# yondonfu/ai-rtc-agent

Measured on NVIDIA H100. Metric: frames/sec at 512x512 SD-Turbo img2img (1-step, stream-batch 1), higher is better.
Workload: dtype f16

## Files before the change

### ai-rtc-agent_b200/csrc/ptx.cuh

```cuda
#pragma once
#include <cuda.h>
#include <cuda_fp16.h>
#include <cuda_runtime.h>
#include <stdint.h>
#include <stdio.h>

namespace b2 {

__device__ __forceinline__ uint32_t smem_u32(const void* p) {
    return static_cast<uint32_t>(__cvta_generic_to_shared(p));
}

__device__ __forceinline__ uint64_t globaltimer_ns() {
    uint64_t t;
    asm volatile("mov.u64 %0, %%globaltimer;" : "=l"(t));
    return t;
}

__device__ __forceinline__ void mbar_init(uint64_t* bar, uint32_t count) {
    asm volatile("mbarrier.init.shared::cta.b64 [%0], %1;" ::"r"(smem_u32(bar)), "r"(count));
}
__device__ __forceinline__ void fence_mbar_init() {
    asm volatile("fence.mbarrier_init.release.cluster;" ::: "memory");
}
__device__ __forceinline__ void mbar_expect_tx(uint64_t* bar, uint32_t bytes) {
    asm volatile("mbarrier.arrive.expect_tx.shared::cta.b64 _, [%0], %1;" ::"r"(smem_u32(bar)),
                 "r"(bytes)
                 : "memory");
}
__device__ __forceinline__ void mbar_arrive(uint64_t* bar) {
    asm volatile("mbarrier.arrive.shared::cta.b64 _, [%0];" ::"r"(smem_u32(bar)) : "memory");
}
__device__ __forceinline__ bool mbar_try_wait(uint64_t* bar, uint32_t parity) {
    uint32_t ok;
    asm volatile(
        "{\n\t"
        ".reg .pred P;\n\t"
        "mbarrier.try_wait.parity.shared::cta.b64 P, [%1], %2;\n\t"
        "selp.u32 %0, 1, 0, P;\n\t"
        "}\n"
        : "=r"(ok)
        : "r"(smem_u32(bar)), "r"(parity)
        : "memory");
    return ok != 0;
}
#ifndef B2_WAIT_TIMEOUT_NS
#define B2_WAIT_TIMEOUT_NS 4000000000ull
#endif
__device__ __forceinline__ void mbar_wait(uint64_t* bar, uint32_t parity) {
    if (mbar_try_wait(bar, parity)) return;
    uint64_t t0 = 0;
    uint32_t spins = 0;
    while (!mbar_try_wait(bar, parity)) {
        if ((++spins & 0x3ff) == 0) {
            const uint64_t now = globaltimer_ns();
            if (t0 == 0) t0 = now;
            else if (now - t0 > B2_WAIT_TIMEOUT_NS) __trap();
        }
    }
}

__device__ __forceinline__ void mbar_arrive_remote(uint32_t cluster_addr) {
    asm volatile("mbarrier.arrive.shared::cluster.b64 _, [%0];" ::"r"(cluster_addr) : "memory");
}

__device__ __forceinline__ void fence_proxy_async_smem() {
    asm volatile("fence.proxy.async.shared::cta;" ::: "memory");
}

__device__ __forceinline__ void cluster_sync_all() {
    asm volatile("barrier.cluster.arrive.release.aligned;" ::: "memory");
    asm volatile("barrier.cluster.wait.acquire.aligned;" ::: "memory");
}
__device__ __forceinline__ void cluster_arrive_relaxed() { asm volatile("barrier.cluster.arrive.relaxed.aligned;" ::: "memory"); }
__device__ __forceinline__ void cluster_wait() { asm volatile("barrier.cluster.wait.aligned;" ::: "memory"); }
__device__ __forceinline__ uint32_t cluster_ctarank() {
    uint32_t r;
    asm volatile("mov.u32 %0, %%cluster_ctarank;" : "=r"(r));
    return r;
}
__device__ __forceinline__ uint32_t dsmem_map(uint32_t local_smem_addr, uint32_t rank) {
    uint32_t r;
    asm volatile("mapa.shared::cluster.u32 %0, %1, %2;" : "=r"(r) : "r"(local_smem_addr), "r"(rank));
    return r;
}
__device__ __forceinline__ void dsmem_st_f2(uint32_t cluster_addr, float x, float y) {
    asm volatile("st.shared::cluster.v2.f32 [%0], {%1, %2};" ::"r"(cluster_addr), "f"(x), "f"(y) : "memory");
}
__device__ __forceinline__ float4 dsmem_ld_f4(uint32_t cluster_addr) {
    float4 v;
    asm volatile("ld.shared::cluster.v4.f32 {%0, %1, %2, %3}, [%4];"
                 : "=f"(v.x), "=f"(v.y), "=f"(v.z), "=f"(v.w)
                 : "r"(cluster_addr)
                 : "memory");
    return v;
}

__device__ __forceinline__ void tma_prefetch_desc(const CUtensorMap* m) {
    asm volatile("prefetch.tensormap [%0];" ::"l"(reinterpret_cast<uint64_t>(m)) : "memory");
}
__device__ __forceinline__ void tma_load_2d(void* smem_dst, const CUtensorMap* m, uint64_t* bar,
                                            int c0, int c1) {
    asm volatile(
        "cp.async.bulk.tensor.2d.shared::cluster.global.mbarrier::complete_tx::bytes [%0], [%1, {%3, "
        "%4}], [%2];" ::"r"(smem_u32(smem_dst)),
        "l"(reinterpret_cast<uint64_t>(m)), "r"(smem_u32(bar)), "r"(c0), "r"(c1)
        : "memory");
}
__device__ __forceinline__ void tma_load_4d(void* smem_dst, const CUtensorMap* m, uint64_t* bar,
                                            int c0, int c1, int c2, int c3) {
    asm volatile(
        "cp.async.bulk.tensor.4d.shared::cluster.global.mbarrier::complete_tx::bytes [%0], [%1, {%3, "
        "%4, %5, %6}], [%2];" ::"r"(smem_u32(smem_dst)),
        "l"(reinterpret_cast<uint64_t>(m)), "r"(smem_u32(bar)), "r"(c0), "r"(c1), "r"(c2), "r"(c3)
        : "memory");
}

__device__ __forceinline__ void tma_load_2d_mc(void* smem_dst, const CUtensorMap* m, uint64_t* bar, int c0, int c1, uint16_t cta_mask) {
    asm volatile(
        "cp.async.bulk.tensor.2d.shared::cluster.global.mbarrier::complete_tx::bytes.multicast::cluster [%0], [%1, {%3, %4}], [%2], "
        "%5;" ::"r"(smem_u32(smem_dst)),
        "l"(reinterpret_cast<uint64_t>(m)), "r"(smem_u32(bar)), "r"(c0), "r"(c1), "h"(cta_mask)
        : "memory");
}

__device__ __forceinline__ void wgmma_fence() { asm volatile("wgmma.fence.sync.aligned;" ::: "memory"); }
__device__ __forceinline__ void wgmma_commit() { asm volatile("wgmma.commit_group.sync.aligned;" ::: "memory"); }
template <int N>
__device__ __forceinline__ void wgmma_wait() { asm volatile("wgmma.wait_group.sync.aligned %0;" ::"n"(N) : "memory"); }
template <int N>
__device__ __forceinline__ void wgmma_fence_regs(float (&d)[N]) {
#pragma unroll
    for (int i = 0; i < N; ++i) asm volatile("" : "+f"(d[i])::"memory");
}

__device__ __forceinline__ uint64_t make_kmajor_sw128_desc(uint32_t smem_addr, uint32_t sbo = 1024) {
    uint64_t d = 0;
    d |= (uint64_t)((smem_addr & 0x3ffff) >> 4);
    d |= (uint64_t)1 << 16;
    d |= (uint64_t)(sbo >> 4) << 32;
    d |= (uint64_t)1 << 62;
    return d;
}

}
```

### ai-rtc-agent_b200/csrc/tconv.cu

```cuda
#include "tconv.cuh"

#include <cudaTypedefs.h>
#include <stdlib.h>

#include "epilogue.cuh"
#include "launch.cuh"
#include "ptx.cuh"

namespace b2 {

constexpr uint32_t TC_WTILE = TC_C * TC_C * 2;
constexpr uint32_t TC_HALO_BYTES = (TC_TW + 2) * (TC_TH + 2) * TC_C * 2;

__global__ void __launch_bounds__(TC_THREADS, 1) tconv_kernel(const __grid_constant__ TconvParams p) {
    extern __shared__ uint8_t smem_raw[];
    uint8_t* smem = reinterpret_cast<uint8_t*>((reinterpret_cast<uintptr_t>(smem_raw) + 1023) & ~static_cast<uintptr_t>(1023));
    const int warp = threadIdx.x >> 5;
    const int lane = threadIdx.x & 31;
    uint8_t* sW = smem;
    uint8_t* sA = smem + 9 * TC_WTILE;
    uint64_t* w_full = reinterpret_cast<uint64_t*>(sA + (size_t)p.nbuf * p.abuf_bytes);
    uint64_t* a_full = w_full + 1;
    uint64_t* a_empty = a_full + TC_MAX_ABUF;

    if (threadIdx.x == TC_CONS) {
        tma_prefetch_desc(&p.tmA);
        tma_prefetch_desc(&p.tmB);
        mbar_init(w_full, 1);
        for (int s = 0; s < p.nbuf; ++s) {
            mbar_init(&a_full[s], 1);
            mbar_init(&a_empty[s], 4);
        }
        fence_mbar_init();
    }
    __syncthreads();
    if (threadIdx.x == TC_CONS) {
        mbar_expect_tx(w_full, 9 * TC_WTILE);
        for (int tap = 0; tap < 9; ++tap) tma_load_2d(sW + tap * TC_WTILE, &p.tmB, w_full, tap * TC_C, 0);
    }
    pdl_launch_dependents();
    pdl_wait();

    const int tiles_per_img = p.tiles_w * p.tiles_h;
    if (warp == TC_CONS / 32) {
        if (lane == 0) {
            int slot = 0;
            uint32_t phase = 0;
            for (int mt = blockIdx.x; mt < p.num_tiles; mt += gridDim.x) {
                const int tiw = mt % p.tiles_w, tih = (mt / p.tiles_w) % p.tiles_h, n0 = mt / tiles_per_img;
                mbar_wait(&a_empty[slot], phase ^ 1);
                mbar_expect_tx(&a_full[slot], TC_HALO_BYTES);
                tma_load_4d(sA + (size_t)slot * p.abuf_bytes, &p.tmA, &a_full[slot], 0, tiw * TC_TW - 1, tih * TC_TH - 1, n0);
                if (++slot == p.nbuf) {
                    slot = 0;
                    phase ^= 1;
                }
            }
        }
    } else {
        const int wg = warp >> 2;
        const uint32_t sa_base = smem_u32(sA);
        const uint64_t db0 = make_kmajor_sw128_desc(smem_u32(sW));
        constexpr int pitch = TC_TW + 2;
        const int rq = (warp & 3) * 16 + (lane >> 2);
        const IgEpilogue& e = p.epi;
        mbar_wait(w_full, 0);
        for (int it = wg, mt = blockIdx.x + wg * gridDim.x; mt < p.num_tiles; it += 2, mt += 2 * gridDim.x) {
            const int slot = it % p.nbuf;
            mbar_wait(&a_full[slot], (uint32_t)(it / p.nbuf) & 1u);
            float acc[2][TC_C / 2];
#pragma unroll
            for (int m = 0; m < 2; ++m)
#pragma unroll
                for (int i = 0; i < TC_C / 2; ++i) acc[m][i] = 0.f;
            wgmma_fence_regs(acc[0]);
            wgmma_fence_regs(acc[1]);
            wgmma_fence();
            const uint32_t a0 = sa_base + (uint32_t)slot * p.abuf_bytes;
#pragma unroll
            for (int tap = 0; tap < 9; ++tap) {
                const uint64_t db = db0 + (uint64_t)(tap * (TC_WTILE >> 4));
#pragma unroll
                for (int m = 0; m < 2; ++m) {
                    const uint32_t sa = a0 + (uint32_t)((8 * m + tap / 3) * pitch + tap % 3) * 128u;
                    const uint64_t da = make_kmajor_sw128_desc(sa, pitch * 128);
#pragma unroll
                    for (int k = 0; k < 4; ++k) Wgmma<TC_C>::ss(acc[m], da + 2 * k, db + 2 * k, 1u);
                }
            }
            wgmma_commit();
            wgmma_wait<0>();
            wgmma_fence_regs(acc[0]);
            wgmma_fence_regs(acc[1]);
            if (lane == 0) mbar_arrive(&a_empty[slot]);
            const int tiw = mt % p.tiles_w, tih = (mt / p.tiles_w) % p.tiles_h, n0 = mt / tiles_per_img;
#pragma unroll
            for (int m = 0; m < 2; ++m) {
                EpiRow rw[2];
#pragma unroll
                for (int h = 0; h < 2; ++h) {
                    const int r = 64 * m + rq + 8 * h;
                    const int hh = tih * TC_TH + (r >> 3), ww = tiw * TC_TW + (r & 7);
                    rw[h].ok = (hh < p.Ho) && (ww < p.Wo);
                    rw[h].orow = ((long)n0 * p.Ho + hh) * p.Wo + ww;
                    rw[h].b = n0;
                    rw[h].mu = 0.f;
                    rw[h].rstd = 1.f;
                }
                epi_frag<TC_C>(e, acc[m], rw, 0, false, lane);
            }
        }
    }
}

bool tconv_eligible(const IgemmDesc& d) {
    const IgEpilogue& e = d.epi;
    return d.nseg == 1 && d.ntap[0] == 9 && d.stride <= 1 && !d.swap && d.src[0].C == TC_C && e.n_valid == TC_C &&
           d.w_rows >= TC_C && d.w_ld == 9 * TC_C && d.src[0].H == d.Ho && d.src[0].W == d.Wo && d.src[0].N == d.Nb &&
           !(e.flags & (IG_GEGLU | IG_SPLITK | IG_SILU)) && (e.ldc & 7) == 0 && (!e.res || (e.ldr & 7) == 0) && (e.colbias_bstride & 3) == 0 &&
           (d.src[0].ld & 7) == 0 && !(reinterpret_cast<uintptr_t>(d.src[0].ptr) & 15) && !(reinterpret_cast<uintptr_t>(d.w) & 15) &&
           !(reinterpret_cast<uintptr_t>(e.out) & 15) && !(reinterpret_cast<uintptr_t>(e.res) & 15) &&
           !(reinterpret_cast<uintptr_t>(e.colbias) & 15);
}

int igemm_encode_act_map(CUtensorMap* m, const ActView& a, int box_c, int box_w, int box_h, int box_n, int estride);
int igemm_encode_w_map(CUtensorMap* m, const __half* w, int rows, int ld, int box_rows);

int tconv_plan(const IgemmDesc& d, TconvPlan* plan) {
    *plan = TconvPlan{};
    if (!tconv_eligible(d)) {
        b2_set_error("tconv: needs a stride-1 3x3 convolution with 64 input and 64 output channels and a vectorisable epilogue");
        return -1;
    }
    TconvParams& p = plan->p;
    p.tiles_w = (d.Wo + TC_TW - 1) / TC_TW;
    p.tiles_h = (d.Ho + TC_TH - 1) / TC_TH;
    p.num_tiles = p.tiles_w * p.tiles_h * d.Nb;
    p.Wo = d.Wo; p.Ho = d.Ho; p.Nb = d.Nb;
    static const char* nb_env = getenv("B2_TCONV_NBUF");
    p.nbuf = nb_env ? atoi(nb_env) : 4;
    if (p.nbuf < 2) p.nbuf = 2;
    if (p.nbuf > TC_MAX_ABUF) p.nbuf = TC_MAX_ABUF;
    p.nbuf &= ~1;
    p.abuf_bytes = (TC_HALO_BYTES + 1023u) & ~1023u;
    p.epi = d.epi;
    if (igemm_encode_act_map(&p.tmA, d.src[0], TC_C, TC_TW + 2, TC_TH + 2, 1, 1)) return -1;
    if (igemm_encode_w_map(&p.tmB, d.w, d.w_rows, d.w_ld, TC_C)) return -1;
    const int sms = b2_device_sms();
    plan->grid = dim3(p.num_tiles < sms ? p.num_tiles : sms, 1, 1);
    plan->smem = 9 * (size_t)TC_WTILE + (size_t)p.nbuf * p.abuf_bytes + 1024  + 512 ;
    plan->rows_total = (long)d.Nb * d.Ho * d.Wo;
    return 0;
}

int tconv_init() {
    static bool done = false;
    if (!done) {
        cudaError_t e = cudaFuncSetAttribute(tconv_kernel, cudaFuncAttributeMaxDynamicSharedMemorySize, 227 * 1024);
        if (e != cudaSuccess) {
            b2_set_error("cudaFuncSetAttribute(tconv): %s", cudaGetErrorString(e));
            return -1;
        }
        done = true;
    }
    return 0;
}

int tconv_launch(const TconvPlan& plan, cudaStream_t stream) {
    if (tconv_init()) return -1;
    cudaError_t e = launch_k(tconv_kernel, plan.grid, dim3(TC_THREADS), plan.smem, stream, 1, plan.p);
    if (e != cudaSuccess) {
        b2_set_error("tconv launch: %s", cudaGetErrorString(e));
        return -1;
    }
    return 0;
}

}
```

### ai-rtc-agent_b200/csrc/tconv.cuh

```cuda
#pragma once
#include "igemm.cuh"

namespace b2 {

constexpr int TC_CONS = 256;
constexpr int TC_THREADS = TC_CONS + 32;
constexpr int TC_TW = 8, TC_TH = 16;
constexpr int TC_C = 64;
constexpr int TC_MAX_ABUF = 6;

struct TconvParams {
    CUtensorMap tmA;
    CUtensorMap tmB;
    int tiles_w, tiles_h, num_tiles;
    int Wo, Ho, Nb;
    int nbuf;
    uint32_t abuf_bytes;
    IgEpilogue epi;
};

struct TconvPlan {
    TconvParams p;
    dim3 grid;
    size_t smem;
    long rows_total;
};

bool tconv_eligible(const IgemmDesc& d);
int tconv_plan(const IgemmDesc& d, TconvPlan* plan);
int tconv_launch(const TconvPlan& plan, cudaStream_t stream);
int tconv_init();

}
```

Measured before the change: 173.0.

## Stage tconv epilogue through swizzled smem and write via TMA stores with residual TMA loads

Replaces the per-thread global epilogue of the 64-channel 3x3 conv kernel with a staged epilogue: fragments are written into swizzled shared memory, the residual tile is fetched by TMA into the same staging buffer, and output is written back with 4D TMA bulk stores. The wgmma loop is reordered so each half-tile commits separately, letting the first half's epilogue overlap the second half's MMAs. It also narrows eligibility (no per-batch bias, colsum, rowstat or second output) and caps A buffers at 4 to fit the staging space. This targets uncoalesced global stores and residual loads, at the cost of extra shared memory, named barriers and fewer A pipeline stages.

```diff
diff --git a/ai-rtc-agent_b200/csrc/ptx.cuh b/ai-rtc-agent_b200/csrc/ptx.cuh
--- a/ai-rtc-agent_b200/csrc/ptx.cuh
+++ b/ai-rtc-agent_b200/csrc/ptx.cuh
@@ -116,6 +116,21 @@
         : "memory");
 }
 
+__device__ __forceinline__ void tma_store_4d(const CUtensorMap* m, const void* smem_src, int c0, int c1, int c2, int c3) {
+    asm volatile("cp.async.bulk.tensor.4d.global.shared::cta.bulk_group [%0, {%2, %3, %4, %5}], [%1];" ::"l"(reinterpret_cast<uint64_t>(m)),
+                 "r"(smem_u32(smem_src)), "r"(c0), "r"(c1), "r"(c2), "r"(c3)
+                 : "memory");
+}
+__device__ __forceinline__ void bulk_commit_group() { asm volatile("cp.async.bulk.commit_group;" ::: "memory"); }
+template <int N>
+__device__ __forceinline__ void bulk_wait_group_read() { asm volatile("cp.async.bulk.wait_group.read %0;" ::"n"(N) : "memory"); }
+template <int N>
+__device__ __forceinline__ void bulk_wait_group() { asm volatile("cp.async.bulk.wait_group %0;" ::"n"(N) : "memory"); }
+
+__device__ __forceinline__ void named_bar_sync(int id, int count) {
+    asm volatile("bar.sync %0, %1;" ::"r"(id), "r"(count) : "memory");
+}
+
 __device__ __forceinline__ void tma_load_2d_mc(void* smem_dst, const CUtensorMap* m, uint64_t* bar, int c0, int c1, uint16_t cta_mask) {
     asm volatile(
         "cp.async.bulk.tensor.2d.shared::cluster.global.mbarrier::complete_tx::bytes.multicast::cluster [%0], [%1, {%3, %4}], [%2], "
diff --git a/ai-rtc-agent_b200/csrc/tconv.cu b/ai-rtc-agent_b200/csrc/tconv.cu
--- a/ai-rtc-agent_b200/csrc/tconv.cu
+++ b/ai-rtc-agent_b200/csrc/tconv.cu
@@ -3,34 +3,42 @@
 #include <cudaTypedefs.h>
 #include <stdlib.h>
 
-#include "epilogue.cuh"
 #include "launch.cuh"
 #include "ptx.cuh"
+#include "wgmma.cuh"
 
 namespace b2 {
 
 constexpr uint32_t TC_WTILE = TC_C * TC_C * 2;
 constexpr uint32_t TC_HALO_BYTES = (TC_TW + 2) * (TC_TH + 2) * TC_C * 2;
+constexpr uint32_t TC_SLAB_BYTES = 64 * TC_C * 2;
+constexpr uint32_t TC_STG_BYTES = 2 * TC_SLAB_BYTES;
 
 __global__ void __launch_bounds__(TC_THREADS, 1) tconv_kernel(const __grid_constant__ TconvParams p) {
     extern __shared__ uint8_t smem_raw[];
-    uint8_t* smem = reinterpret_cast<uint8_t*>((reinterpret_cast<uintptr_t>(smem_raw) + 1023) & ~static_cast<uintptr_t>(1023));
+    uint8_t* smem = smem_raw + ((1024u - (smem_u32(smem_raw) & 1023u)) & 1023u);
     const int warp = threadIdx.x >> 5;
     const int lane = threadIdx.x & 31;
     uint8_t* sW = smem;
     uint8_t* sA = smem + 9 * TC_WTILE;
-    uint64_t* w_full = reinterpret_cast<uint64_t*>(sA + (size_t)p.nbuf * p.abuf_bytes);
+    uint8_t* sS = sA + (size_t)p.nbuf * p.abuf_bytes;
+    uint64_t* w_full = reinterpret_cast<uint64_t*>(sS + 2 * TC_STG_BYTES);
     uint64_t* a_full = w_full + 1;
     uint64_t* a_empty = a_full + TC_MAX_ABUF;
+    uint64_t* r_full = a_empty + TC_MAX_ABUF;
 
     if (threadIdx.x == TC_CONS) {
         tma_prefetch_desc(&p.tmA);
         tma_prefetch_desc(&p.tmB);
+        tma_prefetch_desc(&p.tmO);
+        if (p.epi.res) tma_prefetch_desc(&p.tmR);
         mbar_init(w_full, 1);
         for (int s = 0; s < p.nbuf; ++s) {
             mbar_init(&a_full[s], 1);
             mbar_init(&a_empty[s], 4);
         }
+        mbar_init(&r_full[0], 1);
+        mbar_init(&r_full[1], 1);
         fence_mbar_init();
     }
     __syncthreads();
@@ -59,13 +67,25 @@
         }
     } else {
         const int wg = warp >> 2;
+        const bool leader = (threadIdx.x & 127) == 0;
         const uint32_t sa_base = smem_u32(sA);
         const uint64_t db0 = make_kmajor_sw128_desc(smem_u32(sW));
         constexpr int pitch = TC_TW + 2;
         const int rq = (warp & 3) * 16 + (lane >> 2);
         const IgEpilogue& e = p.epi;
+        const bool has_bias = e.colbias != nullptr, has_res = e.res != nullptr, relu = (e.flags & IG_RELU) != 0;
+        float bias[TC_C / 4];
+#pragma unroll
+        for (int j = 0; j < TC_C / 8; ++j) {
+            const float2 b = has_bias ? *reinterpret_cast<const float2*>(e.colbias + 8 * j + 2 * (lane & 3)) : make_float2(0.f, 0.f);
+            bias[2 * j] = b.x;
+            bias[2 * j + 1] = b.y;
+        }
+        uint8_t* stg = sS + wg * TC_STG_BYTES;
+        uint8_t* stg_t = stg + rq * 128 + 4 * (lane & 3);
         mbar_wait(w_full, 0);
         for (int it = wg, mt = blockIdx.x + wg * gridDim.x; mt < p.num_tiles; it += 2, mt += 2 * gridDim.x) {
+            const int tiw = mt % p.tiles_w, tih = (mt / p.tiles_w) % p.tiles_h, n0 = mt / tiles_per_img;
             const int slot = it % p.nbuf;
             mbar_wait(&a_full[slot], (uint32_t)(it / p.nbuf) & 1u);
             float acc[2][TC_C / 2];
@@ -78,38 +98,72 @@
             wgmma_fence();
             const uint32_t a0 = sa_base + (uint32_t)slot * p.abuf_bytes;
 #pragma unroll
-            for (int tap = 0; tap < 9; ++tap) {
-                const uint64_t db = db0 + (uint64_t)(tap * (TC_WTILE >> 4));
-#pragma unroll
-                for (int m = 0; m < 2; ++m) {
+            for (int m = 0; m < 2; ++m) {
+#pragma unroll
+                for (int tap = 0; tap < 9; ++tap) {
+                    const uint64_t db = db0 + (uint64_t)(tap * (TC_WTILE >> 4));
                     const uint32_t sa = a0 + (uint32_t)((8 * m + tap / 3) * pitch + tap % 3) * 128u;
                     const uint64_t da = make_kmajor_sw128_desc(sa, pitch * 128);
 #pragma unroll
                     for (int k = 0; k < 4; ++k) Wgmma<TC_C>::ss(acc[m], da + 2 * k, db + 2 * k, 1u);
                 }
-            }
-            wgmma_commit();
-            wgmma_wait<0>();
-            wgmma_fence_regs(acc[0]);
-            wgmma_fence_regs(acc[1]);
-            if (lane == 0) mbar_arrive(&a_empty[slot]);
-            const int tiw = mt % p.tiles_w, tih = (mt / p.tiles_w) % p.tiles_h, n0 = mt / tiles_per_img;
+                wgmma_commit();
+            }
+            if (leader) {
+                bulk_wait_group_read<0>();
+                if (has_res) {
+                    mbar_expect_tx(&r_full[wg], TC_STG_BYTES);
+                    tma_load_4d(stg, &p.tmR, &r_full[wg], 0, tiw * TC_TW, tih * TC_TH, n0);
+                } else {
+                    mbar_arrive(&r_full[wg]);
+                }
+            }
 #pragma unroll
             for (int m = 0; m < 2; ++m) {
-                EpiRow rw[2];
-#pragma unroll
-                for (int h = 0; h < 2; ++h) {
-                    const int r = 64 * m + rq + 8 * h;
-                    const int hh = tih * TC_TH + (r >> 3), ww = tiw * TC_TW + (r & 7);
-                    rw[h].ok = (hh < p.Ho) && (ww < p.Wo);
-                    rw[h].orow = ((long)n0 * p.Ho + hh) * p.Wo + ww;
-                    rw[h].b = n0;
-                    rw[h].mu = 0.f;
-                    rw[h].rstd = 1.f;
-                }
-                epi_frag<TC_C>(e, acc[m], rw, 0, false, lane);
-            }
-        }
+                if (m == 0) {
+                    wgmma_wait<1>();
+                    wgmma_fence_regs(acc[0]);
+                    mbar_wait(&r_full[wg], (uint32_t)(it >> 1) & 1u);
+                } else {
+                    wgmma_wait<0>();
+                    wgmma_fence_regs(acc[1]);
+                    if (lane == 0) mbar_arrive(&a_empty[slot]);
+                }
+#pragma unroll
+                for (int j = 0; j < TC_C / 8; ++j) {
+#pragma unroll
+                    for (int h = 0; h < 2; ++h) {
+                        __half2* sp = reinterpret_cast<__half2*>(stg_t + (64 * m + 8 * h) * 128 + ((j ^ (lane >> 2)) << 4));
+                        float x0 = acc[m][4 * j + 2 * h], x1 = acc[m][4 * j + 2 * h + 1];
+                        if (has_bias) {
+                            x0 += bias[2 * j];
+                            x1 += bias[2 * j + 1];
+                        }
+                        if (e.acc_scale != 1.0f) {
+                            x0 *= e.acc_scale;
+                            x1 *= e.acc_scale;
+                        }
+                        if (has_res) {
+                            const float2 f = __half22float2(*sp);
+                            x0 = fmaf(e.res_scale, f.x, x0);
+                            x1 = fmaf(e.res_scale, f.y, x1);
+                        }
+                        if (relu) {
+                            x0 = fmaxf(x0, 0.f);
+                            x1 = fmaxf(x1, 0.f);
+                        }
+                        *sp = __floats2half2_rn(x0, x1);
+                    }
+                }
+                fence_proxy_async_smem();
+                named_bar_sync(1 + wg, 128);
+                if (leader) {
+                    tma_store_4d(&p.tmO, stg + m * TC_SLAB_BYTES, 0, tiw * TC_TW, tih * TC_TH + 8 * m, n0);
+                    bulk_commit_group();
+                }
+            }
+        }
+        if (leader) bulk_wait_group<0>();
     }
 }
 
@@ -117,7 +171,8 @@
     const IgEpilogue& e = d.epi;
     return d.nseg == 1 && d.ntap[0] == 9 && d.stride <= 1 && !d.swap && d.src[0].C == TC_C && e.n_valid == TC_C &&
            d.w_rows >= TC_C && d.w_ld == 9 * TC_C && d.src[0].H == d.Ho && d.src[0].W == d.Wo && d.src[0].N == d.Nb &&
-           !(e.flags & (IG_GEGLU | IG_SPLITK | IG_SILU)) && (e.ldc & 7) == 0 && (!e.res || (e.ldr & 7) == 0) && (e.colbias_bstride & 3) == 0 &&
+           !(e.flags & (IG_GEGLU | IG_SPLITK | IG_SILU)) && !e.colsum && !e.rowstat_out && !e.out2 && (e.ldc & 7) == 0 &&
+           (!e.res || (e.ldr & 7) == 0) && e.colbias_bstride == 0 &&
            (d.src[0].ld & 7) == 0 && !(reinterpret_cast<uintptr_t>(d.src[0].ptr) & 15) && !(reinterpret_cast<uintptr_t>(d.w) & 15) &&
            !(reinterpret_cast<uintptr_t>(e.out) & 15) && !(reinterpret_cast<uintptr_t>(e.res) & 15) &&
            !(reinterpret_cast<uintptr_t>(e.colbias) & 15);
@@ -129,7 +184,8 @@
 int tconv_plan(const IgemmDesc& d, TconvPlan* plan) {
     *plan = TconvPlan{};
     if (!tconv_eligible(d)) {
-        b2_set_error("tconv: needs a stride-1 3x3 convolution with 64 input and 64 output channels and a vectorisable epilogue");
+        b2_set_error("tconv: needs a stride-1 3x3 convolution with 64 input and 64 output channels, 16-byte-aligned pitches and an "
+                     "epilogue of a batch-shared bias / scale / residual / ReLU");
         return -1;
     }
     TconvParams& p = plan->p;
@@ -138,7 +194,7 @@
     p.num_tiles = p.tiles_w * p.tiles_h * d.Nb;
     p.Wo = d.Wo; p.Ho = d.Ho; p.Nb = d.Nb;
     static const char* nb_env = getenv("B2_TCONV_NBUF");
-    p.nbuf = nb_env ? atoi(nb_env) : 4;
+    p.nbuf = nb_env ? atoi(nb_env) : TC_MAX_ABUF;
     if (p.nbuf < 2) p.nbuf = 2;
     if (p.nbuf > TC_MAX_ABUF) p.nbuf = TC_MAX_ABUF;
     p.nbuf &= ~1;
@@ -146,9 +202,16 @@
     p.epi = d.epi;
     if (igemm_encode_act_map(&p.tmA, d.src[0], TC_C, TC_TW + 2, TC_TH + 2, 1, 1)) return -1;
     if (igemm_encode_w_map(&p.tmB, d.w, d.w_rows, d.w_ld, TC_C)) return -1;
+    const ActView out{d.epi.out, d.Nb, d.Ho, d.Wo, TC_C, d.epi.ldc};
+    if (igemm_encode_act_map(&p.tmO, out, TC_C, TC_TW, TC_TH / 2, 1, 1)) return -1;
+    if (d.epi.res) {
+        const ActView res{d.epi.res, d.Nb, d.Ho, d.Wo, TC_C, d.epi.ldr};
+        if (igemm_encode_act_map(&p.tmR, res, TC_C, TC_TW, TC_TH, 1, 1)) return -1;
+    }
     const int sms = b2_device_sms();
     plan->grid = dim3(p.num_tiles < sms ? p.num_tiles : sms, 1, 1);
-    plan->smem = 9 * (size_t)TC_WTILE + (size_t)p.nbuf * p.abuf_bytes + 1024  + 512 ;
+    plan->smem = 9 * (size_t)TC_WTILE + (size_t)p.nbuf * p.abuf_bytes + 2 * (size_t)TC_STG_BYTES + 1024  +
+                 512 ;
     plan->rows_total = (long)d.Nb * d.Ho * d.Wo;
     return 0;
 }
diff --git a/ai-rtc-agent_b200/csrc/tconv.cuh b/ai-rtc-agent_b200/csrc/tconv.cuh
--- a/ai-rtc-agent_b200/csrc/tconv.cuh
+++ b/ai-rtc-agent_b200/csrc/tconv.cuh
@@ -7,11 +7,13 @@
 constexpr int TC_THREADS = TC_CONS + 32;
 constexpr int TC_TW = 8, TC_TH = 16;
 constexpr int TC_C = 64;
-constexpr int TC_MAX_ABUF = 6;
+constexpr int TC_MAX_ABUF = 4;
 
 struct TconvParams {
     CUtensorMap tmA;
     CUtensorMap tmB;
+    CUtensorMap tmO;
+    CUtensorMap tmR;
     int tiles_w, tiles_h, num_tiles;
     int Wo, Ho, Nb;
     int nbuf;
```

Result: faster. 197.7, median of 6 (+14.3%).
